# wolearyc/ramannoodle

Hardware: AMD Instinct MI355X
Metric: structures/sec (GNN polarizability eval) (higher is better)
Workload: dtype f32

## Files before the change

### ramannoodle_amd/csrc/api.hip

```cpp
#include <hip/hip_runtime.h>

#include <algorithm>
#include <chrono>
#include <cmath>
#include <cstdarg>
#include <cstdio>
#include <cstdlib>
#include <cstring>
#include <functional>
#include <memory>
#include <mutex>
#include <string>
#include <thread>
#include <vector>

#include "../../include/rn_potgnn.h"
#include "kernels.hpp"

using namespace rn;

namespace {

std::string g_create_error;

// ... 625 lines not shown
  HIP_TRY(hipMemcpy(P.lattice.p, lat, sizeof(lat), hipMemcpyHostToDevice));
  T *w = P.weights.template as<T>();
  P.pass.resize(L.pass.size());
  for (size_t p = 0; p < L.pass.size(); ++p) {
    const auto &q = L.pass[p];
    PassW<T> &o = P.pass[p];
    o.c1_WnT = w + q.c1_WnT;
    o.c1_WeT = w + q.c1_WeT;
    o.c1_bias = w + q.c1_bias;
    o.c1_norm = {w + q.c1n_g, w + q.c1n_b};
    o.final_norm = {w + q.fin_g, w + q.fin_b};
    o.c2_WT = w + q.c2_WT;
    o.c2_bias = w + q.c2_bias;
    o.c2_norm_1 = {w + q.c2n1_g, w + q.c2n1_b};
    o.c2_norm_2 = {w + q.c2n2_g, w + q.c2n2_b};
    o.c3_WnT = w + q.c3_WnT;
    o.c3_nshift = w + q.c3_nshift;
    o.c3_WeT = w + q.c3_WeT;
    o.c3_norm_1 = {w + q.c3n1_g, w + q.c3n1_b};
    o.c3_norm_2 = {w + q.c3n2_g, w + q.c3n2_b};
    o.c3_norm_1s = {w + q.c3n1_gs, w + q.c3n1_bs};
    o.c2_norm_1s = {w + q.c2n1_gs, w + q.c2n1_bs};
    o.c1_norm_s = {w + q.c1n_gs, w + q.c1n_bs};
    o.mfma_scale = w + q.mfma_scale;
    o.c3_WeT_c = w + q.c3_WeT_c;
    o.c3_WnT_c = w + q.c3_WnT_c;
    o.c3_nshift_c = w + q.c3_nshift_c;
    o.c2_WT_c = w + q.c2_WT_c;
    o.c2_bias_c = w + q.c2_bias_c;
    o.mfma_scale_c = w + q.mfma_scale_c;
    o.c1_WnT_c = w + q.c1_WnT_c;
    o.c1_WeT_c = w + q.c1_WeT_c;
    o.c1_bias_c = w + q.c1_bias_c;
  }
  refresh_pass_flags<T>(h);
  P.ro = {w + L.W0T, w + L.scale0, w + L.shift0, w + L.W3T, w + L.b3, w + L.W5T, w + L.b5, w + L.ro_mfma_scale};
  P.offsets = w + L.offsets;
  P.node_table = w + L.node_table;
  P.ones = w + L.ones;

  const size_t N = h->cfg.num_atoms, E = h->cfg.num_edges, S = chunk_frames<T>(h);
  const size_t FnP = h->d.FnP, FeP = h->d.FeP;
  const bool lean = sizeof(T) == 4 && lean_workspace(h);
  const size_t bufA = bufA_width(h, lean);
  for (int l = 0; l < h->num_lanes; ++l) {
    Lane<T> &ln = P.lanes[l];
    HIP_TRY(hipStreamCreateWithFlags(&ln.stream, hipStreamNonBlocking));
    HIP_TRY(hipEventCreateWithFlags(&ln.done, hipEventDisableTiming));
    ln.unit4.ensure(S * E * 4 * sizeof(T));
    for (int i = 0; i < 2; ++i) {
      ln.node[i].ensure(S * N * FnP * sizeof(T));
      ln.edge[i].ensure(S * E * FeP * sizeof(T));
    }
    ln.npc1.ensure(S * N * 2 * FnP * sizeof(T));
    ln.np3.ensure(S * N * 6 * FeP * sizeof(T));
    ln.bufA.ensure(S * E * bufA * sizeof(T));
    if (!lean) ln.bufB.ensure(S * E * 4 * FeP * sizeof(T));
    if (sizeof(T) == 4 && (h->use_edge2 || h->use_edge3)) ln.c2.ensure(S * E * FeP * sizeof(T));
  }
  if (h->keep_stages) {
    const int np = h->cfg.num_message_passes + 1;
    P.snap_node.resize(np);
    P.snap_edge.resize(np);
    for (int i = 0; i < np; ++i) {
      P.snap_node[i].ensure(S * N * FnP * sizeof(T));
      P.snap_edge[i].ensure(S * E * FeP * sizeof(T));
    }
  }
  launch_setup<T>(w + L.emb, w + L.W2, w + L.b2, w + L.W4, w + L.b4, h->cfg.num_atom_types, h->d,
                  w + L.node_table, w + L.b0, w + L.bn_w, w + L.bn_b, w + L.bn_rm, w + L.bn_rv,
                  w + L.scale0, w + L.shift0, P.lanes[0].stream);
  HIP_TRY(hipGetLastError());
  HIP_TRY(hipStreamSynchronize(P.lanes[0].stream));
  P.ready = true;
}

struct Timer {
  rn_potgnn *h;
  hipStream_t st;
  int kid;
  hipEvent_t a = nullptr, b = nullptr;
  bool on;
  Timer(rn_potgnn *h_, hipStream_t st_, int kid_) : h(h_), st(st_), kid(kid_) {
    on = h->profiling == 1 || (h->profiling >= 100 && h->profiling < 1000 && h->profiling - 100 == kid) ||
         (h->profiling >= 1000 && (((h->profiling - 1000) >> kid) & 1));
    if (on) {
      HIP_TRY(hipEventCreate(&a));
      HIP_TRY(hipEventCreate(&b));
      HIP_TRY(hipEventRecord(a, st));
    }
  }
  ~Timer() noexcept(false) {
    if (on) {
      (void)hipEventRecord(b, st);
      h->timed.push_back({kid, a, b});
    }
    if (h->debug_sync) {
      hipError_t e = hipGetLastError();
      if (e == hipSuccess) e = hipStreamSynchronize(st);
      if (e != hipSuccess) throw HipError{e, kKernelNames[kid]};
    }
  }
};

void resolve_timers(rn_potgnn *h) {
  for (auto &t : h->timed) {
    float ms = 0;
    if (hipEventSynchronize(t.b) == hipSuccess && hipEventElapsedTime(&ms, t.a, t.b) == hipSuccess) {
      h->k_ms[t.kid] += ms;
      h->k_launches[t.kid] += 1;
    }
    (void)hipEventDestroy(t.a);
    (void)hipEventDestroy(t.b);
  }
  h->timed.clear();
}

template <typename T>
struct ChunkRun {
  rn_potgnn *h;
  Lane<T> *ln;
  const double *d_pos;
  const float *d_pos32 = nullptr;
  int S;
  double *d_alpha;
  float *d_vec6;
  double *d_alpha_raw;
  const T *d_lat = nullptr;
  const int *d_types = nullptr;
  int cur = 0;
  T *node[2], *edge[2], *unit4, *npc1, *np3, *bufA, *bufB, *c2;
  int64_t MN, ME;

  ChunkRun(rn_potgnn *h_, Lane<T> &l, const double *pos, int S_, double *alpha, float *vec6,
           double *alpha_raw)
      : h(h_), ln(&l), d_pos(pos), S(S_), d_alpha(alpha), d_vec6(vec6), d_alpha_raw(alpha_raw) {
    node[0] = l.node[0].template as<T>();
    node[1] = l.node[1].template as<T>();
    edge[0] = l.edge[0].template as<T>();
    edge[1] = l.edge[1].template as<T>();
    unit4 = l.unit4.template as<T>();
    npc1 = l.npc1.template as<T>();
    np3 = l.np3.template as<T>();
    bufA = l.bufA.template as<T>();
    bufB = l.bufB.template as<T>();
    c2 = l.c2.template as<T>();
    MN = (int64_t)S * h->g.N;
    ME = (int64_t)S * h->g.E;
  }
  hipStream_t st() const { return ln->stream; }
  void target_tape(int slot, int which) {
    Precision<T> &P = prec<T>(h);
    if (!P.tape_on) return;
    node[which] = P.tape_node[slot].template as<T>();
    edge[which] = P.tape_edge[slot].template as<T>();
  }
  void snapshot(int p) {
    Precision<T> &P = prec<T>(h);
    if (!h->keep_stages) return;
    HIP_TRY(hipMemcpyAsync(P.snap_node[p].p, node[cur], (size_t)MN * h->d.FnP * sizeof(T),
                           hipMemcpyDeviceToDevice, st()));
    HIP_TRY(hipMemcpyAsync(P.snap_edge[p].p, edge[cur], (size_t)ME * h->d.FeP * sizeof(T),
                           hipMemcpyDeviceToDevice, st()));
  }

  void begin() {
    Precision<T> &P = prec<T>(h);
    target_tape(0, 0);
    {
      Timer t(h, st(), K_GEOM);
      bool done = false;
      if constexpr (sizeof(T) == 4) {
        if (d_pos32) {
          const float *lat = d_lat ? d_lat : P.lattice.template as<T>();
          if (pair_rows()) launch_geom_rbf_pairs_pos32(d_pos32, S, h->g, lat, d_lat ? 9 : 0, P.offsets, (T)h->cfg.gauss_coefficient, h->d, unit4, edge[0], st());
          else launch_geom_rbf_pos32(d_pos32, S, h->g, lat, d_lat ? 9 : 0, P.offsets, (T)h->cfg.gauss_coefficient, h->d, unit4, edge[0], st(), narrow());
          done = true;
        } else if (pair_rows()) {
          launch_geom_rbf_pairs(d_pos, S, h->g, d_lat ? d_lat : P.lattice.template as<T>(), d_lat ? 9 : 0, P.offsets,
                                (T)h->cfg.gauss_coefficient, h->d, unit4, edge[0], st());
          done = true;
        }
      }
      if (!done)
        launch_geom_rbf<T>(d_pos, S, h->g, d_lat ? d_lat : P.lattice.template as<T>(), d_lat ? 9 : 0,
                           P.offsets, (T)h->cfg.gauss_coefficient, h->d, unit4, edge[0], st(), narrow());
      h->last_in_order = narrow();
    }
    {
      Timer t(h, st(), K_NODE_INIT);
      launch_node_init<T>(P.node_table, S, h->g, h->d, node[0], d_types, st());
    }
    cur = 0;
    snapshot(0);
  }

  void stage_project(int p) {
    const PassW<T> &w = prec<T>(h).pass[p];
    const Graph &g = h->g;
    const Dims d = h->d;
    const int nxt = cur ^ 1;
    target_tape(p + 1, nxt);
    auto project = [&](const T *X, int64_t R, int K, const T *WT, int NOUT, T *Y, const T *bias, int amode, const T *nd) {
      if constexpr (sizeof(T) == 4) {
        if (h->mfma_f16 && h->split_projections &&
            launch_rowgemm_split(X, K, K, R, WT, NOUT, Y, false, bias, amode, nd, g, st()))
          return;
      }
      launch_rowgemm<T>(X, R, K, WT, NOUT, Y, nullptr, bias, false, amode, nd, g, st());
    };
    if constexpr (sizeof(T) == 4) {
      if (narrow()) {
        Timer t(h, st(), K_NODE_AGG);
        launch_node_narrow(edge[cur], node[cur], node[nxt], S, g, d, w, st());
        return;
      }
    }
    {
      Timer t(h, st(), K_PROJ_NODE);
      if (node_centred()) project(node[cur], MN, d.FnP, w.c1_WnT_c, 2 * d.FnP, npc1, w.c1_bias_c, 0, nullptr);
      else project(node[cur], MN, d.FnP, w.c1_WnT, 2 * d.FnP, npc1, w.c1_bias, 0, nullptr);
    }
    bool node_fused = false;
    if constexpr (sizeof(T) == 4) {
      if (fused() && h->use_node_fused) {
        Timer t(h, st(), K_NODE_AGG);
        if (node_centred() && g.na_num > 0) launch_node_atom(edge[cur], node[cur], npc1, node[nxt], S, g, d, w, st(), pair_rows());
        else launch_node_fused(edge[cur], node[cur], npc1, node[nxt], S, g, d, w, h->mfma_f16, node_centred(), st());
        node_fused = true;
      }
    }
    if (!node_fused) {
      {
        Timer t(h, st(), K_PROJ_EDGE_C1);
        project(edge[cur], ME, d.FeP, w.c1_WeT, 2 * d.FnP, bufA, nullptr, 0, nullptr);
      }
      {
        Timer t(h, st(), K_NODE_AGG);
        launch_node_agg<T>(npc1, bufA, node[cur], node[nxt], S, g, d, w, st());
      }
    }
    {
      Timer t(h, st(), K_PROJ_NODE);
      if (role_split(w)) project(node[nxt], MN, d.FnP, w.c3_WnT_c, 6 * d.FeP, np3, w.c3_nshift_c, 0, nullptr);
      else project(node[nxt], MN, d.FnP, w.c3_WnT, 6 * d.FeP, np3, w.c3_nshift, 0, nullptr);
    }
    if constexpr (sizeof(T) == 4) {
#if RN_EXPERIMENTS
      if (fused() && (h->use_edge2 || (h->use_edge3 && edge3_applicable(w, h->mfma_f16)))) {
        Timer t(h, st(), K_PROJ_C2);
        launch_edge_c2(node[nxt], c2, S, g, d, w, h->mfma_f16, st());
      }
#endif
    }
    if (!fused()) {
      {
        Timer t(h, st(), K_PROJ_EDGE_C3);
        project(edge[cur], ME, d.FeP, w.c3_WeT, 4 * d.FeP, bufB, nullptr, 0, nullptr);
      }
      {
        Timer t(h, st(), K_PROJ_C2);
        project(nullptr, ME, d.FnP, w.c2_WT, 2 * d.FeP, bufA, w.c2_bias, 1, node[nxt]);
      }
    }
  }

  void stage_aggregate(int p) {
    const PassW<T> &w = prec<T>(h).pass[p];
    const int nxt = cur ^ 1;
    {
      Timer t(h, st(), K_EDGE_AGG);
      if constexpr (sizeof(T) == 4) {
        if (narrow()) launch_edge_narrow(edge[cur], edge[nxt], node[nxt], S, h->g, h->d, w, st());
#if RN_EXPERIMENTS
        else if (fused() && h->use_edge3 && edge3_applicable(w, h->mfma_f16))
          launch_edge3(edge[cur], edge[nxt], np3, c2, tape_agg(p), S, h->g, h->d, w, st());
        else if (fused() && h->use_edge2)
          launch_edge2(edge[cur], edge[nxt], np3, c2, tape_agg(p), S, h->g, h->d, w, h->mfma_f16, st());
#endif
        else if (role_split(w)) launch_edge_ps(edge[cur], edge[nxt], node[nxt], np3, tape_agg(p), S, h->g, h->d, w, h->ps_fail.as<int>(), st(), pair_rows(), h->mfma_f16);
// ... 218 lines not shown
                   d_vec6 ? d_vec6 + done * 6 : nullptr, d_alpha_raw ? d_alpha_raw + done * 9 : nullptr,
                   d_lat ? d_lat + done * 9 : nullptr, d_types ? d_types + done * N : nullptr,
                   d_pos32 ? d_pos32 + done * N * 3 : nullptr);
      h->last_chunk_structs = s;
      done += s;
    }
  }
  h->last_was_f64 = sizeof(T) == 8;
  for (int l = 0; l < lanes; ++l) {
    HIP_TRY(hipEventRecord(P.lanes[l].done, P.lanes[l].stream));
    HIP_TRY(hipStreamWaitEvent(user, P.lanes[l].done, 0));
  }
  if (sync) {
    HIP_TRY(hipStreamSynchronize(user));
    resolve_timers(h);
    check_ps_fail(h);
  }
}

template <typename T>
struct Reverse {
  int S, B;
  const T *d_dout6;
  double *d_dpos;
  T *grad;
  bool train_bn;
  double *in_dpos = nullptr;
  double *in_dlat = nullptr;
};

enum { DE0, DE1, DN0, DN1, DNX, DPQ, DNP3, DC2, DPROD, DBC1, DNPC1, DPOL, DUNIT, DH, POL, DOUT, DPROD2, BWN };

template <typename T>
void reverse_pass(rn_potgnn *h, ChunkRun<T> &c, const Reverse<T> &rv) {
  Precision<T> &P = prec<T>(h);
  const PackedLayout &L = h->lay;
  const Graph &g = h->g;
  const Dims d = h->d;
  const int N = g.N, E = g.E, NP = h->cfg.num_message_passes;
  const int S = rv.S, B = rv.B, C = S * B;
  const int HP = std::max(d.FeP, 32);
  hipStream_t st = c.st();
  const size_t ce = (size_t)C * E, cn = (size_t)C * N, fe = (size_t)S * E, fn = (size_t)S * N;
  const size_t sizes[BWN] = {ce * d.FeP, ce * d.FeP, cn * d.FnP, cn * d.FnP, cn * d.FnP,
                             ce * 4 * d.FeP, cn * 6 * d.FeP, ce * std::max(2 * d.FeP, HP), ce * d.FnP,
                             ce * 2 * d.FnP, cn * 2 * d.FnP, ce * 32, ce * 4, ce * HP, fe * 32,
                             (size_t)C * 6, rv.grad ? fe * d.FnP : 0};
  T *b[BWN];
  for (int i = 0; i < BWN; ++i) {
    P.bw[i].ensure(sizes[i] * sizeof(T));
    b[i] = P.bw[i].template as<T>();
  }
  T *bufA = c.bufA, *bufB = c.bufB, *unit4 = c.unit4;
  T *G = rv.grad;
  T *Wd = P.weights.template as<T>();
  const bool split_gemm = sizeof(T) == 4 && h->mfma_f16;
  auto back_gemm = [&](const T *dY, int64_t R, int N, size_t w_off, size_t t_off, int K, T *dX,
                       bool accumulate) {
    if constexpr (sizeof(T) == 4) {
      if (split_gemm && launch_rowgemm_split(dY, N, N, R, Wd + t_off, K, dX, accumulate, nullptr, 0, nullptr, g, st)) return;
      if (launch_rowgemm_blocks(dY, N, N, R, Wd + t_off, K, dX, accumulate, g, st)) return;
    }
    launch_gemm_nt<T>(dY, R, N, Wd + w_off, N, K, dX, accumulate, st);
  };
  auto project = [&](const T *X, int64_t R, int K, const T *WT, int NOUT, T *Y, const T *bias, int amode, const T *node) {
    if constexpr (sizeof(T) == 4) {
      if (split_gemm && launch_rowgemm_split(X, K, K, R, WT, NOUT, Y, false, bias, amode, node, g, st)) return;
    }
    launch_rowgemm<T>(X, R, K, WT, NOUT, Y, nullptr, bias, false, amode, node, g, st);
  };

  TnDeferred tn_store, *tn = nullptr;
  if constexpr (sizeof(T) == 4) {
    static const bool tn_atomic = getenv("RN_POTGNN_TN_ATOMIC") && atoi(getenv("RN_POTGNN_TN_ATOMIC")) != 0;
    if (G && !tn_atomic) {
      size_t need = tn_partial_elems(ce, HP, 32) + tn_partial_elems(ce, HP, HP) + tn_partial_elems(ce, d.FeP, HP);
      const size_t per_pass = tn_partial_elems(ce, d.FeP, 4 * d.FeP) + tn_partial_elems(cn, d.FnP, 6 * d.FeP) +
                              tn_partial_elems(ce, d.FnP, 2 * d.FeP) + tn_partial_elems(ce, d.FeP, 2 * d.FnP) +
                              tn_partial_elems(cn, d.FnP, 2 * d.FnP);
      need += per_pass * (size_t)NP;
      P.tn_arena.ensure(need * sizeof(float));
      tn_store.arena = P.tn_arena.template as<float>();
      tn_store.capacity = need;
      tn = &tn_store;
    }
  }

  static const bool want_side = !(getenv("RN_POTGNN_TN_SIDE") && atoi(getenv("RN_POTGNN_TN_SIDE")) == 0);
  const bool overlap = G != nullptr && sizeof(T) == 4 && want_side;
  hipStream_t sd = st;
  if (overlap) {
    if (!P.side) {
      HIP_TRY(hipStreamCreateWithFlags(&P.side, hipStreamNonBlocking));
      for (auto &e : P.ev_side) HIP_TRY(hipEventCreateWithFlags(&e, hipEventDisableTiming));
    }
    sd = P.side;
  }
  auto side_after_chain = [&](int which) {
    if (!overlap) return;
    HIP_TRY(hipEventRecord(P.ev_side[which], st));
    HIP_TRY(hipStreamWaitEvent(sd, P.ev_side[which], 0));
  };
  auto chain_after_side = [&]() {
    if (!overlap) return;
    HIP_TRY(hipEventRecord(P.ev_side[2], sd));
    HIP_TRY(hipStreamWaitEvent(st, P.ev_side[2], 0));
  };

  const T *edgeP = P.tape_edge[NP].template as<T>();
  if (rv.train_bn) {
    launch_bn_train_apply<T>(P.tape_z1.template as<T>(), fe, HP, d.Fe, P.bn_stats.template as<double>(),
                             h->bn_count, Wd + L.bn_w, Wd + L.bn_b, bufA, b[DH] , st);
  } else {
    launch_rowgemm<T>(edgeP, fe, d.FeP, P.ro.W0T, HP, bufA, P.ro.scale0, P.ro.shift0, true, 0, nullptr, g, st);
  }
  launch_rowgemm<T>(bufA, fe, HP, P.ro.W3T, HP, bufB, P.ones, P.ro.b3, true, 0, nullptr, g, st);
  launch_rowgemm<T>(bufB, fe, HP, P.ro.W5T, 32, b[POL], nullptr, P.ro.b5, false, 0, nullptr, g, st);
  launch_readout_bwd<T>(rv.d_dout6, b[POL], unit4, C, B, g, b[DPOL], b[DUNIT], st);
  if (G) launch_gemm_tn<T>(bufB, HP, b[DPOL], 32, ce, HP, 32, G + L.W5T, 32, G + L.b5, 0, nullptr, g, st, tn);
  back_gemm(b[DPOL], ce, 32, L.W5T, L.t_W5, HP, b[DH], false);
  launch_ssp_bwd<T>(b[DH], bufB, nullptr, E, HP, C, B, st);
  if (G) launch_gemm_tn<T>(bufA, HP, b[DH], HP, ce, HP, HP, G + L.W3T, HP, G + L.b3, 0, nullptr, g, st, tn);
  back_gemm(b[DH], ce, HP, L.W3T, L.t_W3, HP, b[DC2], false);
  if (rv.train_bn) {
    launch_ssp_bwd<T>(b[DC2], bufA, nullptr, E, HP, C, B, st);
    double *stats = P.bn_stats.template as<double>(), *sums = stats + 2 * HP, *own = stats + 4 * HP;
    launch_bn_bwd_sums<T>(b[DC2], P.tape_z1.template as<T>(), fe, HP, d.Fe, stats, h->bn_count, sums, st);
    HIP_TRY(hipMemcpyAsync(own, sums, sizeof(double) * 2 * HP, hipMemcpyDeviceToDevice, st));
    reduce_over_ranks(h, sums, (size_t)2 * HP, st);
    launch_bn_bwd_apply<T>(b[DC2], P.tape_z1.template as<T>(), fe, HP, d.Fe, stats, h->bn_count, sums, own,
                           Wd + L.bn_w, G + L.bn_w, G + L.bn_b, st);
    launch_gemm_tn<T>(edgeP, d.FeP, b[DC2], HP, ce, d.FeP, HP, G + L.W0T, HP, G + L.b0p, 0, nullptr, g, st, tn);
  } else {
    launch_ssp_bwd<T>(b[DC2], bufA, P.ro.scale0, E, HP, C, B, st);
  }
  back_gemm(b[DC2], ce, HP, L.W0T, L.t_W0, d.FeP, b[DE0], false);
  HIP_TRY(hipMemsetAsync(b[DN0], 0, cn * d.FnP * sizeof(T), st));

  int cur = 0;
  for (int p = NP - 1; p >= 0; --p) {
    const PassW<T> &w = P.pass[p];
    PassW<T> gw = w;
    if (G) {
      const auto &q = L.pass[p];
      gw.c1_norm = {G + q.c1n_g, G + q.c1n_b};
      gw.final_norm = {G + q.fin_g, G + q.fin_b};
      gw.c2_norm_1 = {G + q.c2n1_g, G + q.c2n1_b};
      gw.c2_norm_2 = {G + q.c2n2_g, G + q.c2n2_b};
      gw.c3_norm_1 = {G + q.c3n1_g, G + q.c3n1_b};
      gw.c3_norm_2 = {G + q.c3n2_g, G + q.c3n2_b};
    }
    const T *node0 = P.tape_node[p].template as<T>(), *node1 = P.tape_node[p + 1].template as<T>();
    const T *edge0 = P.tape_edge[p].template as<T>(), *edge1 = P.tape_edge[p + 1].template as<T>();
    T *de_next = b[DE0 + cur], *de_prev = b[DE0 + (cur ^ 1)];
    T *dn_next = b[DN0 + cur], *dn_prev = b[DN0 + (cur ^ 1)];
    project(node0, fn, d.FnP, w.c1_WnT, 2 * d.FnP, c.npc1, w.c1_bias, 0, nullptr);
    project(node1, fn, d.FnP, w.c3_WnT, 6 * d.FeP, c.np3, w.c3_nshift, 0, nullptr);
    project(edge0, fe, d.FeP, w.c3_WeT, 4 * d.FeP, bufB, nullptr, 0, nullptr);
    project(nullptr, fe, d.FnP, w.c2_WT, 2 * d.FeP, bufA, w.c2_bias, 1, node1);
    chain_after_side();
    launch_edge_bwd<T>(bufB, c.np3, bufA, edge1, P.tape_agg[p].template as<T>(), de_next, de_prev, b[DPQ],
                       b[DNP3], b[DC2], C, B, g, d, w, G ? &gw : nullptr, st);
    side_after_chain(0);
    back_gemm(b[DPQ], ce, 4 * d.FeP, L.pass[p].c3_WeT, L.pass[p].t_c3We, d.FeP, de_prev, true);
    back_gemm(b[DNP3], cn, 6 * d.FeP, L.pass[p].c3_WnT, L.pass[p].t_c3Wn, d.FnP, dn_next, true);
    back_gemm(b[DC2], ce, 2 * d.FeP, L.pass[p].c2_WT, L.pass[p].t_c2W, d.FnP, b[DPROD], false);
    launch_prod_bwd<T>(b[DPROD], node1, dn_next, C, B, g, d, st);
    if (G) {
      const auto &q = L.pass[p];
      launch_gemm_tn<T>(edge0, d.FeP, b[DPQ], 4 * d.FeP, ce, d.FeP, 4 * d.FeP, G + q.c3_WeT, 4 * d.FeP, nullptr, 0, nullptr, g, sd, tn);
      launch_gemm_tn<T>(node1, d.FnP, b[DNP3], 6 * d.FeP, cn, d.FnP, 6 * d.FeP, G + q.c3_WnT, 6 * d.FeP, G + q.c3_nshift, 0, nullptr, g, sd, tn);
      T *prod = overlap ? b[DPROD2] : b[DPROD];
      launch_prod_fwd<T>(node1, prod, fe, g, d, sd);
      launch_gemm_tn<T>(prod, d.FnP, b[DC2], 2 * d.FeP, ce, d.FnP, 2 * d.FeP, G + q.c2_WT, 2 * d.FeP, G + q.c2_bias, 0, nullptr, g, sd, tn);
    }
    project(edge0, fe, d.FeP, w.c1_WeT, 2 * d.FnP, bufA, nullptr, 0, nullptr);
    launch_node_bwd<T>(c.npc1, bufA, node1, dn_next, dn_prev, b[DBC1], b[DNPC1], C, B, g, d, w,
                       G ? &gw : nullptr, st);
    side_after_chain(1);
    back_gemm(b[DBC1], ce, 2 * d.FnP, L.pass[p].c1_WeT, L.pass[p].t_c1We, d.FeP, de_prev, true);
    back_gemm(b[DNPC1], cn, 2 * d.FnP, L.pass[p].c1_WnT, L.pass[p].t_c1Wn, d.FnP, dn_prev, true);
    if (G) {
      const auto &q = L.pass[p];
      launch_gemm_tn<T>(edge0, d.FeP, b[DBC1], 2 * d.FnP, ce, d.FeP, 2 * d.FnP, G + q.c1_WeT, 2 * d.FnP, nullptr, 0, nullptr, g, sd, tn);
      launch_gemm_tn<T>(node0, d.FnP, b[DNPC1], 2 * d.FnP, cn, d.FnP, 2 * d.FnP, G + q.c1_WnT, 2 * d.FnP, G + q.c1_bias, 0, nullptr, g, sd, tn);
    }
    cur ^= 1;
  }
  chain_after_side();
  if (tn) launch_tn_reduce(*tn, st);
  if (G) {
    P.type_sums.ensure((size_t)h->cfg.num_atom_types * d.Fn * sizeof(T));
    launch_node_embed_bwd<T>(b[DN0 + cur], S, g, d, h->cfg.num_atom_types, Wd + L.emb, Wd + L.W2, Wd + L.b2,
                             Wd + L.W4, G + L.emb, G + L.W2, G + L.b2, G + L.W4, G + L.b4,
                             P.type_sums.template as<T>(), c.d_types, st);
  }
  if (rv.d_dpos)
    launch_geom_bwd<T>(b[DE0 + cur], b[DUNIT], unit4, P.lattice.template as<T>(), P.offsets,
                       (T)h->cfg.gauss_coefficient, C, B, g, d, rv.d_dpos, st);
  if (rv.in_dpos || rv.in_dlat) {
    P.in_dcart.ensure((size_t)C * E * 3 * sizeof(double));
    launch_geom_input_bwd<T>(b[DE0 + cur], b[DUNIT], unit4, c.d_pos, c.d_lat ? c.d_lat : P.lattice.template as<T>(),
                             c.d_lat ? 9 : 0, P.offsets, (T)h->cfg.gauss_coefficient, C, B, g, d,
                             P.in_dcart.template as<double>(), rv.in_dpos, rv.in_dlat, st);
  }
  HIP_TRY(hipGetLastError());
}

template <typename T>
void ensure_tape(rn_potgnn *h, int S) {
  Precision<T> &P = prec<T>(h);
  const int NP = h->cfg.num_message_passes;
  P.tape_node.resize(NP + 1);
  P.tape_edge.resize(NP + 1);
  P.tape_agg.resize(NP + 1);
  for (int p = 0; p <= NP; ++p) {
    P.tape_node[p].ensure((size_t)S * h->g.N * h->d.FnP * sizeof(T));
    P.tape_edge[p].ensure((size_t)S * h->g.E * h->d.FeP * sizeof(T));
    P.tape_agg[p].ensure((size_t)S * h->g.E * h->d.FeP * sizeof(T));
  }
  Lane<T> &ln = P.lanes[0];
  ln.bufA.ensure((size_t)S * h->g.E * bufA_width(h, false) * sizeof(T));
  ln.bufB.ensure((size_t)S * h->g.E * 4 * h->d.FeP * sizeof(T));
}

template <typename T>
ChunkRun<T> taped_forward(rn_potgnn *h, const double *d_pos, int S, const T *d_lat = nullptr, const int *d_types = nullptr) {
  Precision<T> &P = prec<T>(h);
  ensure_tape<T>(h, S);
  P.tape_on = true;
// ... 2151 lines not shown
```

### ramannoodle_amd/csrc/kernels.hpp

```cpp
#pragma once
#include <hip/hip_runtime.h>
#include <algorithm>
#include <cstddef>
#include <cstdint>

namespace rn {

struct Graph {
  int N, E;
  const int *edge_a;
  const int *edge_b;
  const int *out_ptr;
  const int *in_ptr;
  const int *in_edge;
  const int *in_pos;
  const int *atom_type;
  const int *rev_edge;
  int num_tiles;
  const int *tile_begin;
  int max_tile_out_rows;
  int max_tile_in_rows;
  int max_tile_nodes;
  int nt_num;
  const int *nt_begin;
// ... 173 lines not shown
  int num;
};
struct TnDeferred {
  float *arena = nullptr;
  size_t capacity = 0, used = 0;
  TnReduceTable table{};
};
size_t tn_partial_elems(int64_t R, int K, int N);
void launch_tn_reduce(TnDeferred &df, hipStream_t st);
template <typename T>
void launch_gemm_tn(const T *X, int ldx, const T *dY, int ldy, int64_t R, int K, int N, T *dWT,
                    int ldw, T *dbias, int amode, const T *node, const Graph &g, hipStream_t st,
                    TnDeferred *defer = nullptr);
template <typename T>
void launch_bn_col_sums(const T *z, int64_t R, int W, double *stats, hipStream_t st);
template <typename T>
void launch_bn_train_apply(const T *z, int64_t R, int W, int F, const double *stats, double count,
                           const T *gamma, const T *beta, T *h, T *mv, hipStream_t st);
template <typename T>
void launch_bn_bwd_sums(const T *d, const T *z, int64_t R, int W, int F, const double *stats, double count,
                        double *sums, hipStream_t st);
template <typename T>
void launch_bn_bwd_apply(T *d, const T *z, int64_t R, int W, int F, const double *stats, double count,
                         const double *sums, const double *own_sums, const T *gamma, T *dgamma, T *dbeta,
                         hipStream_t st);
template <typename T>
void launch_node_embed_bwd(const T *dnode0, int S, const Graph &g, Dims d, int K, const T *emb,
                           const T *W2, const T *b2, const T *W4, T *demb, T *dW2, T *db2, T *dW4,
                           T *db4, T *type_sums_scratch,
                           const int *types , hipStream_t st);
template <typename T>
void launch_geom_bwd(const T *dedge0, const T *dunit, const T *unit4, const T *lat, const T *offs,
                     T coef, int C, int B, const Graph &g, Dims d, double *dpos, hipStream_t st);
template <typename T>
void launch_geom_input_bwd(const T *dedge0, const T *dunit, const T *unit4, const double *pos, const T *lat,
                           int lat_stride, const T *offs, T coef, int C, int B, const Graph &g, Dims d, double *dcart,
                           double *dpos, double *dlat, hipStream_t st);
template <typename T>
void launch_cast_from_f64(const double *src, T *dst, int64_t n, hipStream_t st);
constexpr int kMaxGroups = 16;

void launch_group_increments(const double *jac, int64_t jac_stride, const double *pos, const double *disp,
                             double disp_scale, int64_t steps, int N, const int *perm, const int *gptr, int G,
                             const double *sigma, double *out, hipStream_t st);

constexpr size_t kFusedLdsBudget = 80 * 1024;
size_t edge_fused_lds_bytes(int tile_out_rows, int tile_in_rows, int tile_nodes);
bool edge_fused_supported(const Graph &g, Dims d);
size_t node_fused_lds_bytes(const Graph &g);
size_t node_fused_lds_bytes(int tile_in_rows, int tile_nodes);
void launch_readout_fused(const float *edge, int64_t M, const ReadoutW<float> &w, float *pol, bool f16,
                          hipStream_t st, bool pair_rows = false, int pol_stride = 32 );
size_t node_atom_lds_bytes(int max_deg);
void launch_node_atom(const float *edge, const float *node_in, const float *npc1, float *node_out, int S, const Graph &g,
                      Dims d, const PassW<float> &w, hipStream_t st, bool pair_rows = false);
void launch_node_fused(const float *edge, const float *node_in, const float *npc1, float *node_out, int S,
                       const Graph &g, Dims d, const PassW<float> &w, bool f16, bool centred, hipStream_t st);
size_t edge_ps_lds_bytes(int tile_out_rows, int tile_in_rows, bool gram);
int edge_ps_ring_tiles(bool gram);
int edge_ps_gram_window();
bool edge_ps_tile_ok(const int *rb, const int *re, int D, int back, int ring, int *window);
void launch_edge_ps(const float *edge_in, float *edge_out, const float *node, const float *np3, float *agg_out, int S,
                    const Graph &g, Dims d, const PassW<float> &w, int *fail, hipStream_t st, bool pair_rows = false,
                    bool f16 = true );

#ifndef RN_EXPERIMENTS
#define RN_EXPERIMENTS 0
#endif
#if RN_EXPERIMENTS
size_t edge_fused_lds_bytes(const Graph &g);
void launch_edge_fused(const float *edge_in, float *edge_out, const float *node, const float *np3,
                       float *agg_out, int S, const Graph &g, Dims d, const PassW<float> &w, bool f16,
                       hipStream_t st);
#ifndef RN_E3_WAVES
#define RN_E3_WAVES 12
#endif
constexpr size_t kEdge3LdsBudget = RN_E3_WAVES <= 4 ? 54272 : (RN_E3_WAVES <= 6 ? 80 : 158) * 1024;
size_t edge3_lds_bytes(int rows, int in_rows, int nodes);
inline int edge3_dests_per_round() { return 4 * RN_E3_WAVES; }
bool edge3_supported(const Graph &g, Dims d);
bool edge3_applicable(const PassW<float> &w, bool f16);
void launch_edge3(const float *edge_in, float *edge_out, const float *np3, const float *c2, float *agg_out, int S,
                  const Graph &g, Dims d, const PassW<float> &w, hipStream_t st);
bool node_fused_wave_tiles();
size_t node_wave_lds_bytes(int tile_in_rows, int tile_nodes);
size_t edge2_lds_bytes(int tile_out_rows, int tile_in_rows, int tile_nodes);
bool edge2_supported(const Graph &g, Dims d);
void launch_edge_c2(const float *node, float *c2, int S, const Graph &g, Dims d, const PassW<float> &w, bool f16,
                    hipStream_t st);
void launch_edge2(const float *edge_in, float *edge_out, const float *np3, const float *c2, float *agg_out, int S,
                  const Graph &g, Dims d, const PassW<float> &w, bool f16, hipStream_t st);
#endif

struct DerivedOp {
  int kind;
  int K, N;
  float scale;
  size_t src, dst;
  int Fe = 0, FeP = 0;
};
void launch_adam(float *w, const float *g, float *m, float *v, const unsigned char *trainable, size_t n,
                 double lr, double beta1, double beta2, double eps, double weight_decay, int64_t step,
                 hipStream_t st, const int *poisoned = nullptr );
void launch_refresh_derived(float *w, const DerivedOp *ops, int num_ops, hipStream_t st);
void launch_gather_segments(const float *w, const long long *seg, int nseg, float *staging, hipStream_t st);
void launch_bn_running(float *running_mean, float *running_var, const float *batch_mean, const float *batch_var,
                       int F, double momentum, double unbias, hipStream_t st);

// ... 13 lines not shown
```

### ramannoodle_amd/csrc/kernels_node_atom.hip

```cpp
#include "fused_common.hpp"
#include <type_traits>

namespace rn {
namespace {
constexpr int NA_D = 4;
static_assert((NA_D & (NA_D - 1)) == 0, "ring slots are addressed with a mask");

struct NodeAtomLds {
  size_t atile, land, part, lnp, tab, total;
};
__host__ __device__ inline NodeAtomLds node_atom_lds(int max_deg) {
  auto up = [](size_t b) { return (b + 15) & ~size_t(15); };
  NodeAtomLds L;
  size_t off = 0;
  L.atile = off; off += (size_t)NA_D * NG * FP * 4;
  L.land = off; off += (size_t)4 * 256 * 16;
  L.part = off; off += (size_t)4 * NG * 4 * 4;
  L.lnp = off; off += (size_t)2 * FP * 4;
  L.tab = off; off += up(((size_t)NG * (size_t)(max_deg > 0 ? max_deg : 1) + NG) * 4);
  L.total = off;
  return L;
}

#ifndef RN_NA_PROBE
#define RN_NA_PROBE 0
#endif
#ifndef RN_NA_WGS
#define RN_NA_WGS 4
#endif

__device__ __forceinline__ float sum_quads(float v) { return sum_xor32(sum_xor16(v)); }
__device__ __forceinline__ void part_put(unsigned buf, int l15, int quad, int wave, float v) {
  if (quad == 0) asm volatile("ds_write_b32 %0, %1" ::"v"(buf + (unsigned)(l15 * 4 + wave) * 4u), "v"(v) : "memory");
}
__device__ __forceinline__ float part_get(unsigned buf, int l15) {
  f32x4 p;
  asm volatile("ds_read_b128 %0, %1\n\ts_waitcnt lgkmcnt(0)" : "=&v"(p) : "v"(buf + (unsigned)l15 * 16u) : "memory");
  return (p[0] + p[1]) + (p[2] + p[3]);
}
__device__ __forceinline__ void wg_barrier() { asm volatile("s_waitcnt lgkmcnt(0)\n\ts_barrier" ::: "memory"); }
}

template <bool PAD, bool PRE>
__global__ __launch_bounds__(256, PRE ? RN_NA_WGS : 3) void node_block_atom_kernel(NodeFusedArgs a) {
  extern __shared__ __attribute__((aligned(16))) unsigned char smem_raw[];
  const Graph &g = a.g;
  const NodeAtomLds L = node_atom_lds(g.na_max_deg);
  float *atile = reinterpret_cast<float *>(smem_raw + L.atile);
  float *land = reinterpret_cast<float *>(smem_raw + L.land);
  float *part = reinterpret_cast<float *>(smem_raw + L.part);
  float *lnp = reinterpret_cast<float *>(smem_raw + L.lnp);
  int *tab = reinterpret_cast<int *>(smem_raw + L.tab);

  const int tid = threadIdx.x, lane = tid & 63;
  const int wave = __builtin_amdgcn_readfirstlane(tid >> 6);
  const int l15 = lane & 15, quad = lane >> 4;
  const int frow = tid >> 4;
  const int fcol = 16 * wave + 4 * quad;
  const unsigned atile_a = lds_addr(atile), lnp_a = lds_addr(lnp), tab_a = lds_addr(tab), part_a = lds_addr(part);
  const unsigned land_a = lds_addr(land) + (unsigned)tid * 16u;
  int logical = blockIdx.x;
  if ((gridDim.x & 7) == 0) logical = (blockIdx.x & 7) * (gridDim.x >> 3) + (blockIdx.x >> 3);
  const int tile = logical % g.na_num;
  const int sg = logical / g.na_num, nsg = gridDim.x / g.na_num;
  const int j0 = tile * NG, natoms = min(NG, g.N - j0);

  int *degs = tab + (size_t)NG * max(g.na_max_deg, 1);
  if (tid < NG) degs[tid] = tid < natoms ? g.in_ptr[j0 + tid + 1] - g.in_ptr[j0 + tid] : 0;
  for (int c = tid; c < 2 * FP; c += 256) lnp[c] = c < FP ? a.w.final_norm.g[c] : a.w.final_norm.b[c - FP];
  __syncthreads();
  int R = 0;
  for (int n = 0; n < NG; ++n) R = max(R, degs[n]);
  R = __builtin_amdgcn_readfirstlane(R);
  for (int idx = tid; idx < R * NG; idx += 256) {
    const int n = idx & 15, r = idx >> 4, dn = degs[n];
    tab[idx] = dn > 0 ? g.in_edge[g.in_ptr[j0 + n] + min(r, dn - 1)] : 0;
  }
  const int deg_own = degs[l15];
  const bool own_valid = l15 < natoms;

  WaveB<true> bW;
  const float s1 = a.w.mfma_scale_c[6];
  bW.load2(a.w.c1_WeT_c, 2 * FP, 16 * wave, FP + 16 * wave, l15, quad, s1);

  float gfm[4], bfm[4], gcm[4], bcm[4];
#pragma unroll
  for (int k = 0; k < 4; ++k) {
    gfm[k] = -kLog2e * a.w.c1_norm.g[fcol + k];
    bfm[k] = -kLog2e * a.w.c1_norm.b[fcol + k];
    gcm[k] = 2.0f * kLog2e * a.w.c1_norm.g[FP + fcol + k];
    bcm[k] = 2.0f * kLog2e * a.w.c1_norm.b[FP + fcol + k];
  }
  const float kClamp = 15.0f * 2.0f * kLog2e;
  const int nvalid = min(max(a.d.Fn - fcol, 0), 4);
  const float inv2n = 1.0f / (float)(2 * a.d.Fn), invn = 1.0f / (float)a.d.Fn;
  const float eps_s = 1e-5f * s1 * s1;
  __syncthreads();
  if (sg >= a.S) return;
  const int nframes = (a.S - sg + nsg - 1) / nsg;

  const int arow = j0 + min(l15, natoms - 1);
  auto seed_ptr = [&](int f, int t) { return a.npc1 + ((int64_t)(sg + f * nsg) * g.N + arow) * (2 * FP) + t * FP + fcol; };
  auto old_ptr = [&](int f) { return a.node_in + ((int64_t)(sg + f * nsg) * g.N + arow) * FP + fcol; };
  f32x4 seed[2];
  {
    const float4 s0 = *reinterpret_cast<const float4 *>(seed_ptr(0, 0)), s1v = *reinterpret_cast<const float4 *>(seed_ptr(0, 1));
    seed[0] = f32x4{s0.x, s0.y, s0.z, s0.w} * s1;
    seed[1] = f32x4{s1v.x, s1v.y, s1v.z, s1v.w} * s1;
    asm volatile("" : "+v"(seed[0]), "+v"(seed[1]));
  }
  auto request_old = [&](int f) { dma16(old_ptr(f), land + (2 + (f & 1)) * 1024 + wave * 256); };
  auto request_frame = [&](int f) {
    dma16(seed_ptr(f, 0), land + wave * 256);
    dma16(seed_ptr(f, 1), land + 1024 + wave * 256);
    request_old(f);
  };

  auto epilogue = [&](int f, const f32x4 &sum, const f32x4 *old_given) {
    part_put(part_a + 2 * 256u, l15, quad, wave, sum_quads((sum[0] + sum[1]) + (sum[2] + sum[3])));
    wg_barrier();
    const float mean = part_get(part_a + 2 * 256u, l15) * invn;
    f32x4 dv = sum - mean;
    if (PAD) {
#pragma unroll
      for (int i = 0; i < 4; ++i)
        if (i >= nvalid) dv[i] = 0.f;
    }
    part_put(part_a + 3 * 256u, l15, quad, wave, sum_quads((dv[0] * dv[0] + dv[1] * dv[1]) + (dv[2] * dv[2] + dv[3] * dv[3])));
    f32x4 fg, fb, oldv;
    lds_read3(lnp_a + (unsigned)fcol * 4u, lnp_a + (unsigned)(FP + fcol) * 4u, land_a + (unsigned)(2 + (f & 1)) * 4096u, fg, fb, oldv);
    if (old_given) oldv = *old_given;
    wg_barrier();
    const float rstd = fast_rsq(part_get(part_a + 3 * 256u, l15) * invn + 1e-5f);
    if (own_valid) {
      float4 out;
      out.x = fast_tanh(oldv[0] + (dv[0] * rstd * fg[0] + fb[0]));
      out.y = fast_tanh(oldv[1] + (dv[1] * rstd * fg[1] + fb[1]));
      out.z = fast_tanh(oldv[2] + (dv[2] * rstd * fg[2] + fb[2]));
      out.w = fast_tanh(oldv[3] + (dv[3] * rstd * fg[3] + fb[3]));
      *reinterpret_cast<float4 *>(a.node_out + ((int64_t)(sg + f * nsg) * g.N + j0 + l15) * FP + fcol) = out;
    }
  };

  if (R == 0) {
    for (int f = 0; f < nframes; ++f) {
      const float4 o = *reinterpret_cast<const float4 *>(old_ptr(f));
      const f32x4 ov = {o.x, o.y, o.z, o.w};
      epilogue(f, f32x4{0.f, 0.f, 0.f, 0.f}, &ov);
    }
    return;
  }

  int ff = 0, fr = 0;
  const int piece = (l15 ^ frow) & 15;
  auto request = [&](int slot) {
    const int e = lds_read1(tab_a + (unsigned)(fr * NG + frow) * 4u);
    const int s = sg + min(ff, nframes - 1) * nsg;
    dma16(a.edge + ((int64_t)s * g.E + e) * FP + 4 * piece, atile + slot * (NG * FP) + wave * 256);
    if (++fr == R) {
      fr = 0;
      ++ff;
    }
  };
  request_old(0);
#pragma unroll
  for (int j = 0; j < NA_D - 1; ++j) request(j);
  asm volatile("s_waitcnt vmcnt(%0)" ::"n"(NA_D - 2) : "memory");
  if (!PRE && !(RN_NA_PROBE & 4)) split_own_pair(atile_a, frow, l15);
  wg_barrier();

  unsigned afrag[4];
#pragma unroll
  for (int j = 0; j < 4; ++j) afrag[j] = atile_a + (unsigned)l15 * (FP * 4) + (unsigned)(((4 * quad + j) ^ l15) & 15) * 16u;
  int r = 0, f = 0;
  f32x4 sum = {0.f, 0.f, 0.f, 0.f};
  auto round = [&](auto slot_tag) {
    constexpr int J = decltype(slot_tag)::value;
    f32x4 acc[2] = {seed[0], seed[1]};
    if (!(RN_NA_PROBE & 1)) {
      f16x8 ah[2], al[2];
      load_pair_a_at<J * NG * FP * 4>(afrag, ah, al);
      bW.product_split(ah, al, acc);
    }
    const unsigned pbuf = part_a + (unsigned)(J & 1) * 256u;
    {
      float q = 0.f;
#pragma unroll
      for (int i = 0; i < 4; ++i) q = fmaf(acc[0][i], acc[0][i], fmaf(acc[1][i], acc[1][i], q));
      part_put(pbuf, l15, quad, wave, sum_quads(q));
    }
    asm volatile("s_waitcnt vmcnt(%0)" ::"n"(NA_D - 3) : "memory");
    if (!PRE && !(RN_NA_PROBE & 4)) split_own_pair(atile_a + (unsigned)(((J + 1) & (NA_D - 1)) * NG * FP) * 4u, frow, l15);
    wg_barrier();
    request((J + NA_D - 1) & (NA_D - 1));
    if (r == 0 && f + 1 < nframes) request_frame(f + 1);
    if (!(RN_NA_PROBE & 2)) {
      const float rstd = fast_rsq(fmaf(part_get(pbuf, l15), inv2n, eps_s));
      f32x4 out;
#pragma unroll
      for (int i = 0; i < 4; ++i) {
        const float e1 = fast_exp2(fmaf(acc[0][i] * rstd, gfm[i], bfm[i]));
        const float yc = __builtin_amdgcn_fmed3f(fmaf(acc[1][i] * rstd, gcm[i], bcm[i]), -kClamp, kClamp);
        const float e2 = fast_exp2(yc);
        const float t = 1.0f + e2;
        out[i] = (e2 - 1.0f) * fast_rcp(fmaf(e1, t, t));
      }
      if (r < deg_own) sum += out;
    } else {
      sum += acc[0] + acc[1];
    }
    if (++r < R) return true;
    epilogue(f, sum, nullptr);
    sum = f32x4{0.f, 0.f, 0.f, 0.f};
    r = 0;
    if (++f == nframes) return false;
    if (R < 3) asm volatile("s_waitcnt vmcnt(0)" ::: "memory");
    f32x4 n0, n1;
    lds_read2(land_a, land_a + 4096u, n0, n1);
    seed[0] = n0 * s1;
    seed[1] = n1 * s1;
    return true;
  };
  static_assert(NA_D == 4, "the round loop is unrolled over a four-slot ring");
  for (;;) {
    if (!round(std::integral_constant<int, 0>{})) break;
    if (!round(std::integral_constant<int, 1>{})) break;
    if (!round(std::integral_constant<int, 2>{})) break;
    if (!round(std::integral_constant<int, 3>{})) break;
  }
  asm volatile("s_waitcnt vmcnt(0)" ::: "memory");
}

size_t node_atom_lds_bytes(int max_deg) { return node_atom_lds(max_deg).total; }

void launch_node_atom(const float *edge, const float *node_in, const float *npc1, float *node_out, int S, const Graph &g,
                      Dims d, const PassW<float> &w, hipStream_t st, bool pair_rows) {
  if (S == 0 || g.N == 0) return;
  NodeFusedArgs a{edge, node_in, npc1, node_out, S, g, d, w};
  const bool pad = d.Fn != d.FnP;
  const size_t lds = node_atom_lds_bytes(g.na_max_deg);
  auto kern = pair_rows ? (pad ? &node_block_atom_kernel<true, true> : &node_block_atom_kernel<false, true>)
                        : (pad ? &node_block_atom_kernel<true, false> : &node_block_atom_kernel<false, false>);
  if (lds > 48 * 1024)
    (void)hipFuncSetAttribute(reinterpret_cast<const void *>(kern), hipFuncAttributeMaxDynamicSharedMemorySize, (int)lds);
  static int cus = 0;
  if (cus == 0) {
    int dev = 0;
    hipDeviceProp_t prop;
    if (hipGetDevice(&dev) == hipSuccess && hipGetDeviceProperties(&prop, dev) == hipSuccess) cus = prop.multiProcessorCount;
    if (cus <= 0) cus = 256;
  }
  int per_cu = 0;
  if (hipOccupancyMaxActiveBlocksPerMultiprocessor(&per_cu, kern, 256, lds) != hipSuccess || per_cu < 1) per_cu = 1;
  per_cu = std::min(per_cu, RN_NA_WGS);
  int nsg = per_cu * cus / g.na_num;
  nsg = nsg < 1 ? 1 : (nsg > S ? S : nsg);
  kern<<<(unsigned)nsg * (unsigned)g.na_num, 256, lds, st>>>(a);
}

}
```

Baseline: 64160.

## Fuse node-centred c1 projection into the per-atom node aggregation kernel

```diff
diff --git a/ramannoodle_amd/csrc/api.hip b/ramannoodle_amd/csrc/api.hip
--- a/ramannoodle_amd/csrc/api.hip
+++ b/ramannoodle_amd/csrc/api.hip
@@ -701,7 +701,6 @@
       ln.node[i].ensure(S * N * FnP * sizeof(T));
       ln.edge[i].ensure(S * E * FeP * sizeof(T));
     }
-    ln.npc1.ensure(S * N * 2 * FnP * sizeof(T));
     ln.np3.ensure(S * N * 6 * FeP * sizeof(T));
     ln.bufA.ensure(S * E * bufA * sizeof(T));
     if (!lean) ln.bufB.ensure(S * E * 4 * FeP * sizeof(T));
@@ -778,7 +777,7 @@
   const T *d_lat = nullptr;
   const int *d_types = nullptr;
   int cur = 0;
-  T *node[2], *edge[2], *unit4, *npc1, *np3, *bufA, *bufB, *c2;
+  T *node[2], *edge[2], *unit4, *np3, *bufA, *bufB, *c2;
   int64_t MN, ME;
 
   ChunkRun(rn_potgnn *h_, Lane<T> &l, const double *pos, int S_, double *alpha, float *vec6,
@@ -789,7 +788,6 @@
     edge[0] = l.edge[0].template as<T>();
     edge[1] = l.edge[1].template as<T>();
     unit4 = l.unit4.template as<T>();
-    npc1 = l.npc1.template as<T>();
     np3 = l.np3.template as<T>();
     bufA = l.bufA.template as<T>();
     bufB = l.bufB.template as<T>();
@@ -798,6 +796,10 @@
     ME = (int64_t)S * h->g.E;
   }
   hipStream_t st() const { return ln->stream; }
+  T *npc1_buf() {
+    ln->npc1.ensure((size_t)chunk_frames<T>(h) * h->cfg.num_atoms * 2 * h->d.FnP * sizeof(T));
+    return ln->npc1.template as<T>();
+  }
   void target_tape(int slot, int which) {
     Precision<T> &P = prec<T>(h);
     if (!P.tape_on) return;
@@ -865,7 +867,10 @@
         return;
       }
     }
-    {
+    const bool node_atom = sizeof(T) == 4 && fused() && h->use_node_fused && node_centred() && g.na_num > 0;
+    T *npc1 = nullptr;
+    if (!node_atom) {
+      npc1 = npc1_buf();
       Timer t(h, st(), K_PROJ_NODE);
       if (node_centred()) project(node[cur], MN, d.FnP, w.c1_WnT_c, 2 * d.FnP, npc1, w.c1_bias_c, 0, nullptr);
       else project(node[cur], MN, d.FnP, w.c1_WnT, 2 * d.FnP, npc1, w.c1_bias, 0, nullptr);
@@ -874,7 +879,7 @@
     if constexpr (sizeof(T) == 4) {
       if (fused() && h->use_node_fused) {
         Timer t(h, st(), K_NODE_AGG);
-        if (node_centred() && g.na_num > 0) launch_node_atom(edge[cur], node[cur], npc1, node[nxt], S, g, d, w, st(), pair_rows());
+        if (node_atom) launch_node_atom(edge[cur], node[cur], node[nxt], S, g, d, w, st(), pair_rows());
         else launch_node_fused(edge[cur], node[cur], npc1, node[nxt], S, g, d, w, h->mfma_f16, node_centred(), st());
         node_fused = true;
       }
@@ -1199,6 +1204,7 @@
     b[i] = P.bw[i].template as<T>();
   }
   T *bufA = c.bufA, *bufB = c.bufB, *unit4 = c.unit4;
+  T *npc1 = c.npc1_buf();
   T *G = rv.grad;
   T *Wd = P.weights.template as<T>();
   const bool split_gemm = sizeof(T) == 4 && h->mfma_f16;
@@ -1301,7 +1307,7 @@
     const T *edge0 = P.tape_edge[p].template as<T>(), *edge1 = P.tape_edge[p + 1].template as<T>();
     T *de_next = b[DE0 + cur], *de_prev = b[DE0 + (cur ^ 1)];
     T *dn_next = b[DN0 + cur], *dn_prev = b[DN0 + (cur ^ 1)];
-    project(node0, fn, d.FnP, w.c1_WnT, 2 * d.FnP, c.npc1, w.c1_bias, 0, nullptr);
+    project(node0, fn, d.FnP, w.c1_WnT, 2 * d.FnP, npc1, w.c1_bias, 0, nullptr);
     project(node1, fn, d.FnP, w.c3_WnT, 6 * d.FeP, c.np3, w.c3_nshift, 0, nullptr);
     project(edge0, fe, d.FeP, w.c3_WeT, 4 * d.FeP, bufB, nullptr, 0, nullptr);
     project(nullptr, fe, d.FnP, w.c2_WT, 2 * d.FeP, bufA, w.c2_bias, 1, node1);
@@ -1322,7 +1328,7 @@
       launch_gemm_tn<T>(prod, d.FnP, b[DC2], 2 * d.FeP, ce, d.FnP, 2 * d.FeP, G + q.c2_WT, 2 * d.FeP, G + q.c2_bias, 0, nullptr, g, sd, tn);
     }
     project(edge0, fe, d.FeP, w.c1_WeT, 2 * d.FnP, bufA, nullptr, 0, nullptr);
-    launch_node_bwd<T>(c.npc1, bufA, node1, dn_next, dn_prev, b[DBC1], b[DNPC1], C, B, g, d, w,
+    launch_node_bwd<T>(npc1, bufA, node1, dn_next, dn_prev, b[DBC1], b[DNPC1], C, B, g, d, w,
                        G ? &gw : nullptr, st);
     side_after_chain(1);
     back_gemm(b[DBC1], ce, 2 * d.FnP, L.pass[p].c1_WeT, L.pass[p].t_c1We, d.FeP, de_prev, true);
diff --git a/ramannoodle_amd/csrc/kernels.hpp b/ramannoodle_amd/csrc/kernels.hpp
--- a/ramannoodle_amd/csrc/kernels.hpp
+++ b/ramannoodle_amd/csrc/kernels.hpp
@@ -249,8 +249,8 @@
 void launch_readout_fused(const float *edge, int64_t M, const ReadoutW<float> &w, float *pol, bool f16,
                           hipStream_t st, bool pair_rows = false, int pol_stride = 32 );
 size_t node_atom_lds_bytes(int max_deg);
-void launch_node_atom(const float *edge, const float *node_in, const float *npc1, float *node_out, int S, const Graph &g,
-                      Dims d, const PassW<float> &w, hipStream_t st, bool pair_rows = false);
+void launch_node_atom(const float *edge, const float *node_in, float *node_out, int S, const Graph &g, Dims d,
+                      const PassW<float> &w, hipStream_t st, bool pair_rows = false);
 void launch_node_fused(const float *edge, const float *node_in, const float *npc1, float *node_out, int S,
                        const Graph &g, Dims d, const PassW<float> &w, bool f16, bool centred, hipStream_t st);
 size_t edge_ps_lds_bytes(int tile_out_rows, int tile_in_rows, bool gram);
diff --git a/ramannoodle_amd/csrc/kernels_node_atom.hip b/ramannoodle_amd/csrc/kernels_node_atom.hip
--- a/ramannoodle_amd/csrc/kernels_node_atom.hip
+++ b/ramannoodle_amd/csrc/kernels_node_atom.hip
@@ -14,9 +14,9 @@
   NodeAtomLds L;
   size_t off = 0;
   L.atile = off; off += (size_t)NA_D * NG * FP * 4;
-  L.land = off; off += (size_t)4 * 256 * 16;
+  L.land = off; off += (size_t)2 * 256 * 16;
   L.part = off; off += (size_t)4 * NG * 4 * 4;
-  L.lnp = off; off += (size_t)2 * FP * 4;
+  L.lnp = off; off += (size_t)4 * FP * 4;
   L.tab = off; off += up(((size_t)NG * (size_t)(max_deg > 0 ? max_deg : 1) + NG) * 4);
   L.total = off;
   return L;
@@ -30,12 +30,20 @@
 #endif
 
 __device__ __forceinline__ float sum_quads(float v) { return sum_xor32(sum_xor16(v)); }
-__device__ __forceinline__ void part_put(unsigned buf, int l15, int quad, int wave, float v) {
-  if (quad == 0) asm volatile("ds_write_b32 %0, %1" ::"v"(buf + (unsigned)(l15 * 4 + wave) * 4u), "v"(v) : "memory");
-}
-__device__ __forceinline__ float part_get(unsigned buf, int l15) {
+__device__ __forceinline__ float max_quads(float v) {
+  const auto r = __builtin_amdgcn_permlane16_swap(__float_as_uint(v), __float_as_uint(v), false, false);
+  v = fmaxf(__uint_as_float(r[0]), __uint_as_float(r[1]));
+  const auto q = __builtin_amdgcn_permlane32_swap(__float_as_uint(v), __float_as_uint(v), false, false);
+  return fmaxf(__uint_as_float(q[0]), __uint_as_float(q[1]));
+}
+template <int BUF>
+__device__ __forceinline__ void part_put(unsigned put, int quad, float v) {
+  if (quad == 0) asm volatile("ds_write_b32 %0, %1 offset:%2" ::"v"(put), "v"(v), "n"(BUF * 256) : "memory");
+}
+template <int BUF>
+__device__ __forceinline__ float part_get(unsigned get) {
   f32x4 p;
-  asm volatile("ds_read_b128 %0, %1\n\ts_waitcnt lgkmcnt(0)" : "=&v"(p) : "v"(buf + (unsigned)l15 * 16u) : "memory");
+  asm volatile("ds_read_b128 %0, %1 offset:%2\n\ts_waitcnt lgkmcnt(0)" : "=&v"(p) : "v"(get), "n"(BUF * 256) : "memory");
   return (p[0] + p[1]) + (p[2] + p[3]);
 }
 __device__ __forceinline__ void wg_barrier() { asm volatile("s_waitcnt lgkmcnt(0)\n\ts_barrier" ::: "memory"); }
@@ -57,7 +65,8 @@
   const int l15 = lane & 15, quad = lane >> 4;
   const int frow = tid >> 4;
   const int fcol = 16 * wave + 4 * quad;
-  const unsigned atile_a = lds_addr(atile), lnp_a = lds_addr(lnp), tab_a = lds_addr(tab), part_a = lds_addr(part);
+  const unsigned atile_a = lds_addr(atile), lnp_a = lds_addr(lnp), tab_a = lds_addr(tab);
+  const unsigned put_a = lds_addr(part) + (unsigned)(l15 * 4 + wave) * 4u, get_a = lds_addr(part) + (unsigned)l15 * 16u;
   const unsigned land_a = lds_addr(land) + (unsigned)tid * 16u;
   int logical = blockIdx.x;
   if ((gridDim.x & 7) == 0) logical = (blockIdx.x & 7) * (gridDim.x >> 3) + (blockIdx.x >> 3);
@@ -67,7 +76,7 @@
 
   int *degs = tab + (size_t)NG * max(g.na_max_deg, 1);
   if (tid < NG) degs[tid] = tid < natoms ? g.in_ptr[j0 + tid + 1] - g.in_ptr[j0 + tid] : 0;
-  for (int c = tid; c < 2 * FP; c += 256) lnp[c] = c < FP ? a.w.final_norm.g[c] : a.w.final_norm.b[c - FP];
+  for (int c = tid; c < 4 * FP; c += 256) lnp[c] = c < FP ? a.w.final_norm.g[c] : c < 2 * FP ? a.w.final_norm.b[c - FP] : a.w.c1_bias_c[c - 2 * FP];
   __syncthreads();
   int R = 0;
   for (int n = 0; n < NG; ++n) R = max(R, degs[n]);
@@ -95,43 +104,96 @@
   const int nvalid = min(max(a.d.Fn - fcol, 0), 4);
   const float inv2n = 1.0f / (float)(2 * a.d.Fn), invn = 1.0f / (float)a.d.Fn;
   const float eps_s = 1e-5f * s1 * s1;
+
+  float wn_s[2], wn_inv[2];
+#pragma unroll
+  for (int t = 0; t < 2; ++t) {
+    const float *grp = a.w.c1_WnT_c + (size_t)(quad * KS) * (2 * FP) + ((t * FP + 16 * wave) & ~31) + l15;
+    float m = 0.f;
+#pragma unroll
+    for (int k = 0; k < KS; ++k) m = fmaxf(m, fmaxf(fabsf(grp[(size_t)k * (2 * FP)]), fabsf(grp[(size_t)k * (2 * FP) + 16])));
+#pragma unroll
+    for (int sft = 1; sft < 64; sft <<= 1) m = fmaxf(m, __shfl_xor(m, sft));
+    wn_s[t] = __int_as_float(__builtin_amdgcn_readfirstlane(__float_as_int(mfma_prescale(m))));
+    wn_inv[t] = __int_as_float(__builtin_amdgcn_readfirstlane(__float_as_int(1.0f / wn_s[t])));
+  }
   __syncthreads();
   if (sg >= a.S) return;
   const int nframes = (a.S - sg + nsg - 1) / nsg;
 
   const int arow = j0 + min(l15, natoms - 1);
-  auto seed_ptr = [&](int f, int t) { return a.npc1 + ((int64_t)(sg + f * nsg) * g.N + arow) * (2 * FP) + t * FP + fcol; };
   auto old_ptr = [&](int f) { return a.node_in + ((int64_t)(sg + f * nsg) * g.N + arow) * FP + fcol; };
+  auto request_old = [&](int f) { dma16(old_ptr(f), land + (f & 1) * 1024 + wave * 256); };
+
   f32x4 seed[2];
-  {
-    const float4 s0 = *reinterpret_cast<const float4 *>(seed_ptr(0, 0)), s1v = *reinterpret_cast<const float4 *>(seed_ptr(0, 1));
-    seed[0] = f32x4{s0.x, s0.y, s0.z, s0.w} * s1;
-    seed[1] = f32x4{s1v.x, s1v.y, s1v.z, s1v.w} * s1;
-    asm volatile("" : "+v"(seed[0]), "+v"(seed[1]));
-  }
-  auto request_old = [&](int f) { dma16(old_ptr(f), land + (2 + (f & 1)) * 1024 + wave * 256); };
-  auto request_frame = [&](int f) {
-    dma16(seed_ptr(f, 0), land + wave * 256);
-    dma16(seed_ptr(f, 1), land + 1024 + wave * 256);
-    request_old(f);
+  auto node_term = [&](int f) {
+    const int ln = launder(lane), lq = ln >> 4, ll = ln & 15;
+    const unsigned row_a = lds_addr(land) + (unsigned)(f & 1) * 4096u + (unsigned)lq * 1024u + (unsigned)ll * 16u;
+    const float *wn_lane = a.w.c1_WnT_c + ((lq * KS) * (2 * FP) + 16 * wave + ll);
+    float sr, inv_sr;
+    {
+      f32x4 u[4];
+      asm volatile(
+          "ds_read_b128 %0, %4\n\tds_read_b128 %1, %4 offset:256\n\tds_read_b128 %2, %4 offset:512\n\t"
+          "ds_read_b128 %3, %4 offset:768\n\ts_waitcnt lgkmcnt(0)"
+          : "=&v"(u[0]), "=&v"(u[1]), "=&v"(u[2]), "=&v"(u[3])
+          : "v"(row_a)
+          : "memory");
+      float m = 0.f;
+#pragma unroll
+      for (int j = 0; j < 4; ++j)
+#pragma unroll
+        for (int i = 0; i < 4; ++i) m = fmaxf(m, fabsf(u[j][i]));
+      sr = mfma_prescale(max_quads(m));
+      inv_sr = 1.0f / sr;
+    }
+    f32x4 acc[2] = {{0.f, 0.f, 0.f, 0.f}, {0.f, 0.f, 0.f, 0.f}};
+#pragma unroll
+    for (int s = 0; s < 2; ++s) {
+      f32x4 u[2];
+      asm volatile("ds_read_b128 %0, %2 offset:%3\n\tds_read_b128 %1, %2 offset:%4\n\ts_waitcnt lgkmcnt(0)"
+                   : "=&v"(u[0]), "=&v"(u[1])
+                   : "v"(row_a), "n"(s * 512), "n"(s * 512 + 256)
+                   : "memory");
+      const float x[8] = {u[0][0] * sr, u[0][1] * sr, u[0][2] * sr, u[0][3] * sr, u[1][0] * sr, u[1][1] * sr, u[1][2] * sr, u[1][3] * sr};
+      f16x8 ah, al;
+      split_f16x8(x, ah, al);
+#pragma unroll
+      for (int t = 0; t < 2; ++t) {
+        float wv[8];
+#pragma unroll
+        for (int j = 0; j < 8; ++j) wv[j] = wn_s[t] * wn_lane[(size_t)(8 * s + j) * (2 * FP) + t * FP];
+        f16x8 wh, wl;
+        split_f16x8(wv, wh, wl);
+        acc[t] = mfma_split3(wh, wl, ah, al, acc[t]);
+        asm volatile("" ::: "memory");
+      }
+    }
+    f32x4 bias[2];
+    asm volatile("ds_read_b128 %0, %2 offset:%3\n\tds_read_b128 %1, %2 offset:%4\n\ts_waitcnt lgkmcnt(0)"
+                 : "=&v"(bias[0]), "=&v"(bias[1])
+                 : "v"(lnp_a + (unsigned)fcol * 4u), "n"(2 * FP * 4), "n"(3 * FP * 4)
+                 : "memory");
+#pragma unroll
+    for (int t = 0; t < 2; ++t) seed[t] = (acc[t] * (wn_inv[t] * inv_sr) + bias[t]) * s1;
   };
 
   auto epilogue = [&](int f, const f32x4 &sum, const f32x4 *old_given) {
-    part_put(part_a + 2 * 256u, l15, quad, wave, sum_quads((sum[0] + sum[1]) + (sum[2] + sum[3])));
+    part_put<2>(put_a, quad, sum_quads((sum[0] + sum[1]) + (sum[2] + sum[3])));
     wg_barrier();
-    const float mean = part_get(part_a + 2 * 256u, l15) * invn;
+    const float mean = part_get<2>(get_a) * invn;
     f32x4 dv = sum - mean;
     if (PAD) {
 #pragma unroll
       for (int i = 0; i < 4; ++i)
         if (i >= nvalid) dv[i] = 0.f;
     }
-    part_put(part_a + 3 * 256u, l15, quad, wave, sum_quads((dv[0] * dv[0] + dv[1] * dv[1]) + (dv[2] * dv[2] + dv[3] * dv[3])));
+    part_put<3>(put_a, quad, sum_quads((dv[0] * dv[0] + dv[1] * dv[1]) + (dv[2] * dv[2] + dv[3] * dv[3])));
     f32x4 fg, fb, oldv;
-    lds_read3(lnp_a + (unsigned)fcol * 4u, lnp_a + (unsigned)(FP + fcol) * 4u, land_a + (unsigned)(2 + (f & 1)) * 4096u, fg, fb, oldv);
+    lds_read3(lnp_a + (unsigned)fcol * 4u, lnp_a + (unsigned)(FP + fcol) * 4u, land_a + (unsigned)(f & 1) * 4096u, fg, fb, oldv);
     if (old_given) oldv = *old_given;
     wg_barrier();
-    const float rstd = fast_rsq(part_get(part_a + 3 * 256u, l15) * invn + 1e-5f);
+    const float rstd = fast_rsq(part_get<3>(get_a) * invn + 1e-5f);
     if (own_valid) {
       float4 out;
       out.x = fast_tanh(oldv[0] + (dv[0] * rstd * fg[0] + fb[0]));
@@ -163,6 +225,10 @@
     }
   };
   request_old(0);
+  asm volatile("s_waitcnt vmcnt(0)" ::: "memory");
+  wg_barrier();
+  node_term(0);
+  asm volatile("" : "+v"(seed[0]), "+v"(seed[1]));
 #pragma unroll
   for (int j = 0; j < NA_D - 1; ++j) request(j);
   asm volatile("s_waitcnt vmcnt(%0)" ::"n"(NA_D - 2) : "memory");
@@ -182,20 +248,19 @@
       load_pair_a_at<J * NG * FP * 4>(afrag, ah, al);
       bW.product_split(ah, al, acc);
     }
-    const unsigned pbuf = part_a + (unsigned)(J & 1) * 256u;
     {
       float q = 0.f;
 #pragma unroll
       for (int i = 0; i < 4; ++i) q = fmaf(acc[0][i], acc[0][i], fmaf(acc[1][i], acc[1][i], q));
-      part_put(pbuf, l15, quad, wave, sum_quads(q));
+      part_put<(J & 1)>(put_a, quad, sum_quads(q));
     }
     asm volatile("s_waitcnt vmcnt(%0)" ::"n"(NA_D - 3) : "memory");
     if (!PRE && !(RN_NA_PROBE & 4)) split_own_pair(atile_a + (unsigned)(((J + 1) & (NA_D - 1)) * NG * FP) * 4u, frow, l15);
     wg_barrier();
     request((J + NA_D - 1) & (NA_D - 1));
-    if (r == 0 && f + 1 < nframes) request_frame(f + 1);
+    if (r == 0 && f + 1 < nframes) request_old(f + 1);
     if (!(RN_NA_PROBE & 2)) {
-      const float rstd = fast_rsq(fmaf(part_get(pbuf, l15), inv2n, eps_s));
+      const float rstd = fast_rsq(fmaf(part_get<(J & 1)>(get_a), inv2n, eps_s));
       f32x4 out;
 #pragma unroll
       for (int i = 0; i < 4; ++i) {
@@ -214,11 +279,11 @@
     sum = f32x4{0.f, 0.f, 0.f, 0.f};
     r = 0;
     if (++f == nframes) return false;
-    if (R < 3) asm volatile("s_waitcnt vmcnt(0)" ::: "memory");
-    f32x4 n0, n1;
-    lds_read2(land_a, land_a + 4096u, n0, n1);
-    seed[0] = n0 * s1;
-    seed[1] = n1 * s1;
+    if (R < 3) {
+      asm volatile("s_waitcnt vmcnt(0)" ::: "memory");
+      wg_barrier();
+    }
+    node_term(f);
     return true;
   };
   static_assert(NA_D == 4, "the round loop is unrolled over a four-slot ring");
@@ -233,10 +298,10 @@
 
 size_t node_atom_lds_bytes(int max_deg) { return node_atom_lds(max_deg).total; }
 
-void launch_node_atom(const float *edge, const float *node_in, const float *npc1, float *node_out, int S, const Graph &g,
-                      Dims d, const PassW<float> &w, hipStream_t st, bool pair_rows) {
+void launch_node_atom(const float *edge, const float *node_in, float *node_out, int S, const Graph &g, Dims d,
+                      const PassW<float> &w, hipStream_t st, bool pair_rows) {
   if (S == 0 || g.N == 0) return;
-  NodeFusedArgs a{edge, node_in, npc1, node_out, S, g, d, w};
+  NodeFusedArgs a{edge, node_in, nullptr, node_out, S, g, d, w};
   const bool pad = d.Fn != d.FnP;
   const size_t lds = node_atom_lds_bytes(g.na_max_deg);
   auto kern = pair_rows ? (pad ? &node_block_atom_kernel<true, true> : &node_block_atom_kernel<false, true>)
```

Result: no change. 64480 (median of 6 runs) (+0.5%).
